# albcab/mfm

Measured on NVIDIA B200. Metric: chain-steps/sec (MALA+flow-MH+FM update), pines 40x40, higher is better.
Workload: dtype f32

## Files before the change

mfm_b200/csrc/flow.cu:

```cuda
#include "internal.h"
#include <limits.h>
#include <string.h>
#include <stdlib.h>
#include "gemm_tf32x3.cuh"
#include "ref_dist.cuh"

namespace mfm {

__constant__ float c_alpha[6] = {(float)(1.0 / 5), (float)(3.0 / 10), (float)(4.0 / 5), (float)(8.0 / 9), 1.0f, 1.0f};
__constant__ float c_beta[6][6] = {
    {(float)(1.0 / 5), 0, 0, 0, 0, 0},
    {(float)(3.0 / 40), (float)(9.0 / 40), 0, 0, 0, 0},
    {(float)(44.0 / 45), (float)(-56.0 / 15), (float)(32.0 / 9), 0, 0, 0},
    {(float)(19372.0 / 6561), (float)(-25360.0 / 2187), (float)(64448.0 / 6561), (float)(-212.0 / 729), 0, 0},
    {(float)(9017.0 / 3168), (float)(-355.0 / 33), (float)(46732.0 / 5247), (float)(49.0 / 176), (float)(-5103.0 / 18656), 0},
    {(float)(35.0 / 384), 0, (float)(500.0 / 1113), (float)(125.0 / 192), (float)(-2187.0 / 6784), (float)(11.0 / 84)}};
__constant__ float c_sol[7] = {(float)(35.0 / 384), 0, (float)(500.0 / 1113), (float)(125.0 / 192),
                               (float)(-2187.0 / 6784), (float)(11.0 / 84), 0};
__constant__ float c_err[7] = {(float)(35.0 / 384 - 1951.0 / 21600), 0, (float)(500.0 / 1113 - 22642.0 / 50085),
                               (float)(125.0 / 192 - 451.0 / 720), (float)(-2187.0 / 6784 - -12231.0 / 42400),
                               (float)(11.0 / 84 - 649.0 / 6300), (float)(-1.0 / 60.0)};
__constant__ float c_mid[7] = {(float)(6025192743.0 / 30085553152.0 / 2), 0, (float)(51252292925.0 / 65400821598.0 / 2),
                               (float)(-2691868925.0 / 45128329728.0 / 2), (float)(187940372067.0 / 1594534317056.0 / 2),
                               (float)(-1776094331.0 / 19743644256.0 / 2), (float)(11237099.0 / 235043384.0 / 2)};

struct EpiFieldV {
    static constexpr bool kRowSum = false;
    float* V; long long ldv; const float* bias; const float* gt; const float* gc; long long ld; float sgn;
    const int* row_map;
    float* amax_out = nullptr; mutable float vmax = 0.0f;
    struct Aux { float bias, gt, gc; int orow; };
    __device__ __forceinline__ Aux load(int row, int col) const {
        const long long o = (long long)row * ld + col;
        Aux a; a.bias = __ldg(bias + col); a.gt = __ldg(gt + o); a.gc = __ldg(gc + o);
        a.orow = row_map ? __ldg(row_map + row) : row;
        return a;
    }
    __device__ __forceinline__ float apply(int, int col, float acc, const Aux& a) const {
        const float v = sgn * (acc + a.bias + a.gt * a.gc);
        V[(long long)a.orow * ldv + col] = v; vmax = fmaxf(vmax, fabsf(v));
        return 0.0f;
    }
    __device__ __forceinline__ float operator()(int row, int col, float acc) const { return apply(row, col, acc, load(row, col)); }
    __device__ __forceinline__ void row_partial(int, int, float) const {}
    __device__ __forceinline__ void at_z(int) {}
    struct Col4 { float4 bias; };
    struct Row4 { float4 gt, gc; int orow; };
    bool vec_ok() const { return aligned16(V) && ldv % 4 == 0 && aligned16(bias) && aligned16(gt) && aligned16(gc) && ld % 4 == 0; }
    __device__ __forceinline__ Col4 load_col4(int col) const { Col4 c; c.bias = ldg4(bias + col); return c; }
    __device__ __forceinline__ Row4 load_row4(int row, int col) const {
        const long long o = (long long)row * ld + col;
        Row4 r; r.gt = ldg4(gt + o); r.gc = ldg4(gc + o); r.orow = row_map ? __ldg(row_map + row) : row;
        return r;
    }
    __device__ __forceinline__ float apply4(int, int col, const float4& acc, const Col4& c, const Row4& r) const {
        float4 v;
        v.x = sgn * (acc.x + c.bias.x + r.gt.x * r.gc.x); v.y = sgn * (acc.y + c.bias.y + r.gt.y * r.gc.y);
        v.z = sgn * (acc.z + c.bias.z + r.gt.z * r.gc.z); v.w = sgn * (acc.w + c.bias.w + r.gt.w * r.gc.w);
        st4(V + (long long)r.orow * ldv + col, v);
        vmax = amax4(vmax, v);
        return 0.0f;
    }
};
struct EpiFieldDiv {
    static constexpr bool kRowSum = true;
    const float* z; const float* gt; const float* hvc; long long ld; float* partial; int n_tiles;
    struct Aux { float z, gt, hvc; };
    __device__ __forceinline__ Aux load(int row, int col) const {
        const long long o = (long long)row * ld + col;
        Aux a; a.z = __ldg(z + o); a.gt = __ldg(gt + o); a.hvc = __ldg(hvc + o);
        return a;
    }
    __device__ __forceinline__ float apply(int, int, float acc, const Aux& a) const { return a.z * (acc + a.gt * a.hvc); }
    __device__ __forceinline__ float operator()(int row, int col, float acc) const { return apply(row, col, acc, load(row, col)); }
    struct Col4 {};
    struct Row4 { float4 z, gt, hvc; };
    bool vec_ok() const { return aligned16(z) && aligned16(gt) && aligned16(hvc) && ld % 4 == 0; }
    __device__ __forceinline__ Col4 load_col4(int) const { return Col4{}; }
    __device__ __forceinline__ Row4 load_row4(int row, int col) const {
        const long long o = (long long)row * ld + col;
        Row4 r; r.z = ldg4(z + o); r.gt = ldg4(gt + o); r.hvc = ldg4(hvc + o);
        return r;
    }
    __device__ __forceinline__ float apply4(int, int, const float4& acc, const Col4&, const Row4& r) const {
        return ((r.z.x * (acc.x + r.gt.x * r.hvc.x) + r.z.y * (acc.y + r.gt.y * r.hvc.y)) +
                (r.z.z * (acc.z + r.gt.z * r.hvc.z) + r.z.w * (acc.w + r.gt.w * r.hvc.w)));
    }
    __device__ __forceinline__ void row_partial(int row, int tile, float s) const { partial[(long long)row * n_tiles + tile] = s; }
    __device__ __forceinline__ void at_z(int) {}
};

int dense(int n, int in, int out, const float* A, long long lda, const float* WT, long long ldwt, const float* bias, int relu,
                 float* C, long long ldc, const float* mask, long long ldm, int mask_div, cudaStream_t st,
                 const int* n_rows_dev, DenseAmax am) {
    GemmShape p{n, out, in, A, lda, WT, ldwt, n_rows_dev};
    p.a_amax = am.a; p.a_amax2 = am.a2; p.a_bound = am.a_bound; p.a_split = am.a_split; p.a_scale_src = am.a_scale_src;
    const bool general = relu > ACT_RELU || am.dact != nullptr || am.mask_mul != 0;
    if (am.out_split && am.w_norm && (am.a || am.a_bound > 0.0f)) {
        auto run = [&](auto e) -> cudaError_t {
            e.alt_amax = am.alt_amax; e.alt_w_norm = am.alt_w_norm; e.alt_bias = am.alt_bias;
            e.amax_out = am.out; e.dact = am.dact; e.lddact = am.lddact; e.mask_mul = am.mask_mul;
            return launch_gemm<true, false>(p, e, st);
        };
        if (general) MFM_CUDA_CHECK(run(EpiStdSA{C, ldc, bias, mask, ldm, nullptr, 0, relu, mask_div, am.out_split, am.a, am.a2, am.a_bound, am.w_norm, am.bias_amax, am.add_bound, am.out_bound}));
        else MFM_CUDA_CHECK(run(EpiStdS{C, ldc, bias, mask, ldm, nullptr, 0, relu, mask_div, am.out_split, am.a, am.a2, am.a_bound, am.w_norm, am.bias_amax, am.add_bound, am.out_bound}));
        return MFM_OK;
// ... 582 lines not shown
                                                           int* __restrict__ n_active, long long* __restrict__ chain_evals) {
    __shared__ int wsum[32];
    __shared__ int total;
    const int per = (n + 1023) / 1024;
    const int b = threadIdx.x * per, e = min(n, b + per);
    int cnt = 0;
    for (int c = b; c < e; ++c) cnt += seg[c] < n_seg;
    const int lane = threadIdx.x & 31, w = threadIdx.x >> 5;
    int inc = cnt;
#pragma unroll
    for (int o = 1; o < 32; o <<= 1) { const int v = __shfl_up_sync(0xffffffffu, inc, o); if (lane >= o) inc += v; }
    if (lane == 31) wsum[w] = inc;
    __syncthreads();
    if (w == 0) {
        int v = wsum[lane], iv = v;
#pragma unroll
        for (int o = 1; o < 32; o <<= 1) { const int u = __shfl_up_sync(0xffffffffu, iv, o); if (lane >= o) iv += u; }
        wsum[lane] = iv - v;
        if (lane == 31) total = iv;
    }
    __syncthreads();
    int pos = wsum[w] + inc - cnt;
    for (int c = b; c < e; ++c) if (seg[c] < n_seg) idx[pos++] = c;
    if (threadIdx.x == 0) { *n_active = total; *chain_evals += 6ll * total; }
}

__global__ void ode_gather_probe_kernel(int n, int d, int H, const int* __restrict__ idx, const int* __restrict__ n_active,
                                        const float* __restrict__ z_full, const float* __restrict__ zw2_full,
                                        const float* __restrict__ zkinv_full, float* __restrict__ z, float* __restrict__ zw2,
                                        float* __restrict__ zkinv) {
    const int r = blockIdx.x;
    if (r >= min(n, *n_active)) return;
    const long long c = idx[r];
    for (int i = threadIdx.x; i < d; i += blockDim.x) {
        z[(long long)r * d + i] = z_full[c * d + i];
        if (zkinv_full) zkinv[(long long)r * d + i] = zkinv_full[c * d + i];
    }
    for (int i = threadIdx.x; i < H; i += blockDim.x) zw2[(long long)r * H + i] = zw2_full[c * H + i];
}

__device__ __forceinline__ float fit_eval(float y0, float y1, float ymid, float dy0, float dy1, float h, float rel) {
    const float a = -2.f * h * dy0 + 2.f * h * dy1 - 8.f * y0 - 8.f * y1 + 16.f * ymid;
    const float b = 5.f * h * dy0 - 3.f * h * dy1 + 18.f * y0 + 14.f * y1 - 32.f * ymid;
    const float c = -4.f * h * dy0 + h * dy1 - 11.f * y0 - 5.f * y1 + 16.f * ymid;
    const float dd = h * dy0;
    return (((a * rel + b) * rel + c) * rel + dd) * rel + y0;
}

}
#include "targets.cuh"
#include "ode_small.cuh"
namespace mfm {

__global__ void ode_finish_kernel(int n, int d, OdeState S, OdeTimes TS, float rtol, float atol, int mxstep) {
    const int lane = threadIdx.x & 31;
    const int c = blockIdx.x * (blockDim.x >> 5) + (threadIdx.x >> 5);
    if (c >= n) return;
    int seg = S.seg[c];
    if (seg >= TS.n_seg) return;
    const float tt = S.t[c], h = S.dt[c];
    const long long o = (long long)c * d;
    float sum = 0.0f;
    for (int i = lane; i < d; i += 32) {
        float ss = 0.0f, se = 0.0f;
#pragma unroll
        for (int j = 0; j < 7; ++j) { const float k = S.kx[j][o + i]; ss += c_sol[j] * k; se += c_err[j] * k; }
        const float y = S.yx[o + i];
        const float y1 = h * ss + y;
        const float r = (h * se) / (atol + rtol * fmaxf(fabsf(y), fabsf(y1)));
        sum += r * r;
    }
    float ssl = 0.0f, sel = 0.0f;
#pragma unroll
    for (int j = 0; j < 7; ++j) { const float k = S.kl[j][c]; ssl += c_sol[j] * k; sel += c_err[j] * k; }
    const float yl = S.yl[c];
    const float yl1 = h * ssl + yl;
    if (lane == 0) { const float r = (h * sel) / (atol + rtol * fmaxf(fabsf(yl), fabsf(yl1))); sum += r * r; }
    sum = warp_sum(sum);
    const float ratio = sqrtf(sum / (float)(d + 1));
    const bool accept = ratio <= 1.0f;
    float new_dt;
    if (isnan(ratio)) new_dt = NAN;
    else if (ratio == 0.0f) new_dt = h * 10.0f;
    else {
        const float dfac = ratio < 1.0f ? 1.0f : 0.2f;
        const float fac = fminf(10.0f, fmaxf(powf(ratio, -0.2f) * 0.9f, dfac));
        new_dt = h * fac;
    }
    if (new_dt < 0.0f) new_dt = 0.0f;
    float t_new = tt;
    if (accept) {
        t_new = tt + h;
        const float t_final = TS.target[TS.n_seg - 1];
        const float rel = (t_final - tt) / (t_new - tt);
        for (int i = lane; i < d; i += 32) {
            float ss = 0.0f, sm = 0.0f;
            float k0 = 0.f, k6 = 0.f;
#pragma unroll
            for (int j = 0; j < 7; ++j) {
                const float k = S.kx[j][o + i]; ss += c_sol[j] * k; sm += c_mid[j] * k;
                if (j == 0) k0 = k; if (j == 6) k6 = k;
            }
            const float y = S.yx[o + i];
            const float y1 = h * ss + y, ymid = y + h * sm;
            S.outx[o + i] = fit_eval(y, y1, ymid, k0, k6, h, rel);
            S.yx[o + i] = y1;
            S.kx[0][o + i] = k6;
        }
        if (lane == 0) {
            float sm = 0.0f;
#pragma unroll
            for (int j = 0; j < 7; ++j) sm += c_mid[j] * S.kl[j][c];
            S.outl[c] = fit_eval(yl, yl1, yl + h * sm, S.kl[0][c], S.kl[6][c], h, rel);
            S.yl[c] = yl1; S.kl[0][c] = S.kl[6][c]; S.t[c] = t_new;
        }
    }
    if (lane == 0) {
        int ic = S.icount[c] + 1;
        const int ntry = S.ntry[c] + 1;
        S.ntry[c] = ntry;
        S.dt[c] = new_dt;
        while (seg < TS.n_seg && !(t_new < TS.target[seg] && ic < mxstep && new_dt > 0.0f)) { ++seg; ic = 0; }
        S.seg[c] = seg; S.icount[c] = ic;
        if (seg < TS.n_seg) atomicAdd(&S.counters[0], 1);
        if (accept) atomicAdd(&S.counters[1], 1);
        atomicAdd(&S.counters[2], 1);
        atomicMax(&S.counters[3], ntry);
    }
}

__global__ void copy_out_kernel(int n, int d, const float* __restrict__ sx, const float* __restrict__ sl,
                                float* __restrict__ y1, float* __restrict__ ldj) {
    const long long i = blockIdx.x * (long long)blockDim.x + threadIdx.x;
    if (i < (long long)n * d) y1[i] = sx[i];
    if (i < n && ldj) ldj[i] = sl[i];
}

__global__ void write_stats_kernel(const int* __restrict__ counters, int n_eval, long long host_chain_evals, int* __restrict__ stats,
                                   int accumulate) {
    if (threadIdx.x == 0) {
        if (n_eval == INT_MIN) n_eval = 2 + 6 * counters[3];
        else if (n_eval < 0) n_eval = -n_eval + 6 * counters[12];
        if (host_chain_evals < 0) host_chain_evals = -host_chain_evals * n_eval;
        const long long ce = *reinterpret_cast<const long long*>(counters + 10) + host_chain_evals;
        long long* out_ce = reinterpret_cast<long long*>(stats + 4);
        if (accumulate) { stats[0] += counters[1]; stats[1] += counters[2]; stats[2] = max(stats[2], counters[3]); stats[3] += n_eval; *out_ce += ce; }
        else { stats[0] = counters[1]; stats[1] = counters[2]; stats[2] = counters[3]; stats[3] = n_eval; *out_ce = ce; stats[6] = 0; stats[7] = 0; }
    }
}

__global__ void ode_loop_cond_kernel(cudaGraphConditionalHandle handle, int* __restrict__ counters, long long max_iter) {
    if (threadIdx.x == 0) {
        const int it = ++counters[12];
        cudaGraphSetConditional(handle, (counters[0] > 0 && it < max_iter) ? 1u : 0u);
    }
}
struct OdeGraphKey {
    mfm_field_t F; mfm_target_t T; mfm_ode_opts_t O; int direction, n, flags; const void *z, *z_compact, *ws, *fb;
};
struct OdeGraphEntry { OdeGraphKey key; cudaGraph_t graph; cudaGraphExec_t exec; int dev; long long max_iter; unsigned long long stamp; bool used; };
static thread_local OdeGraphEntry g_ode_graphs[8];
static thread_local unsigned long long g_ode_graph_stamp = 0;
static int g_ode_small = -1;
static bool ode_small_enabled() {
    if (g_ode_small < 0) { const char* e = getenv("MFM_ODE_SMALL"); g_ode_small = (e && e[0] == '0') ? 0 : 1; }
    return g_ode_small != 0;
}
static int g_ode_graph_mode = -1;
static bool ode_use_graph(long long elements) {
    if (g_ode_graph_mode < 0) {
        const char* e = getenv("MFM_ODE_GRAPH");
        g_ode_graph_mode = (e && e[0] == '0') ? 0 : ((e && e[0] == '1') ? 1 : 2);
    }
    return g_ode_graph_mode == 1 || (g_ode_graph_mode == 2 && elements <= (4ll << 20));
}
// ... 84 lines not shown
    const int d = F.dim, H = F.hidden;
    const float sgn = direction >= 0 ? 1.0f : -1.0f;
    if (O.n_times < 2 || O.n_times > 17) { mfm_set_last_error_msg("n_times must be in [2,17]"); return MFM_ERR_ARG; }
    OdeTimes TS; TS.n_seg = O.n_times - 1;
    for (int k = 1; k < O.n_times; ++k) TS.target[k - 1] = (float)((double)k / (double)(O.n_times - 1));
    if (ode_small_enabled() && small::eligible(F, T, n)) {
        small::Args A;
        A.F = F; A.T = T; A.n = n; A.hutch = z != nullptr ? 1 : 0; A.n_seg = TS.n_seg;
        for (int k = 0; k < 16; ++k) A.target[k] = k < TS.n_seg ? TS.target[k] : 0.0f;
        A.rtol = O.rtol; A.atol = O.atol; A.mxstep = O.mxstep; A.sgn = sgn; A.y0 = y0; A.z = z; A.y1 = y1; A.ldj = ldj; A.counters = S.counters; A.wt = B.wt;
        static bool configured = false;
        if (!configured) {
            MFM_CUDA_CHECK(cudaFuncSetAttribute(small::ode_small_kernel, cudaFuncAttributeMaxDynamicSharedMemorySize, small::SMEM_BYTES));
            configured = true;
        }
        MFM_CUDA_CHECK(cudaMemsetAsync(S.counters, 0, 64 * sizeof(int), st));
        small::ode_small_kernel<<<ceil_div(n, small::CH), small::NTHR, small::SMEM_BYTES, st>>>(A);
        MFM_LAUNCH_CHECK();
        if (stats) { write_stats_kernel<<<1, 32, 0, st>>>(S.counters, INT_MIN, 0, stats, stats_accumulate); MFM_LAUNCH_CHECK(); }
        return MFM_OK;
    }
    int* hflag = host_flag();
    if (!hflag) { mfm_set_last_error_msg("cudaMallocHost failed"); return MFM_ERR_CUDA; }
    int rc;
    const int gE = ceil_div((long long)n * d, 256), gW = ceil_div(n, 8);
    const bool compact = z != nullptr;
    ode_init_kernel<<<max(gE, 1), 256, 0, st>>>(n, d, y0, S, 0.0f, sgn);
    MFM_LAUNCH_CHECK();
    if (z) {
        if ((rc = field_prepare_probe(F, T, n, z, B, st, z_bound))) return rc;
        if (compact) {
            MFM_CUDA_CHECK(cudaMemcpyAsync(S.zw2_full, B.zw2, (size_t)n * H * 4, cudaMemcpyDeviceToDevice, st));
            if (T.kind == MFM_TARGET_PINES)
                MFM_CUDA_CHECK(cudaMemcpyAsync(S.zkinv_full, B.zkinv, (size_t)n * d * 4, cudaMemcpyDeviceToDevice, st));
        }
    }
    int n_eval = 0;
    if ((rc = field_eval(F, T, n, S.xi, S.tf, z, sgn, S.kx[0], S.kl[0], B, st))) return rc; ++n_eval;
    ode_h0_kernel<<<gW, 256, 0, st>>>(n, d, S, O.rtol, O.atol, sgn);
    MFM_LAUNCH_CHECK();
    if ((rc = field_eval(F, T, n, S.xi, S.tf, z, sgn, S.kx[1], S.kl[1], B, st))) return rc; ++n_eval;
    ode_h1_kernel<<<gW, 256, 0, st>>>(n, d, S, O.rtol, O.atol);
    MFM_LAUNCH_CHECK();
    const int* idx = nullptr; const int* nact = nullptr; const float* zc = z;
    if (compact) {
        ode_compact_kernel<<<1, 1024, 0, st>>>(n, TS.n_seg, S.seg, S.idx, S.n_active, reinterpret_cast<long long*>(S.counters + 10));
        MFM_LAUNCH_CHECK();
        idx = S.idx; nact = S.n_active; zc = z_compact;
    }
    const long long max_iter = (long long)TS.n_seg * (long long)O.mxstep + 2;
    float* x_amax = (tc2h::gemm_h16() && B.amax && d % 16 == 0 && n >= 256) ? B.amax + AM_X : nullptr;
    bool stage_vec = d % 4 == 0 && ((reinterpret_cast<uintptr_t>(S.yx) | reinterpret_cast<uintptr_t>(S.xi)) & 15) == 0;
    for (int j = 0; j < 6; ++j) stage_vec = stage_vec && (reinterpret_cast<uintptr_t>(S.kx[j]) & 15) == 0;
    auto rk_iteration = [&](cudaStream_t s) -> int {
        int rc2;
        if (compact) {
            ode_gather_probe_kernel<<<n, 128, 0, s>>>(n, d, H, idx, nact, z, S.zw2_full,
                                                      T.kind == MFM_TARGET_PINES ? S.zkinv_full : nullptr, z_compact, B.zw2, B.zkinv);
            MFM_LAUNCH_CHECK();
        }
        for (int sg = 1; sg <= 6; ++sg) {
            if (stage_vec) ode_stage4_kernel<<<ceil_div((long long)n * (d / 4), 256), 256, 0, s>>>(n, d / 4, sg, S, TS.n_seg, sgn, idx, nact, x_amax);
            else ode_stage_kernel<<<gE, 256, 0, s>>>(n, d, sg, S, TS.n_seg, sgn, idx, nact, x_amax);
            MFM_LAUNCH_CHECK();
            if ((rc2 = field_eval(F, T, n, S.xi, S.tf, zc, sgn, S.kx[sg], S.kl[sg], B, s, nact, idx, x_amax))) return rc2;
        }
        MFM_CUDA_CHECK(cudaMemsetAsync(S.counters, 0, sizeof(int), s));
        ode_finish_kernel<<<gW, 256, 0, s>>>(n, d, S, TS, O.rtol, O.atol, O.mxstep);
        MFM_LAUNCH_CHECK();
        if (compact) {
            ode_compact_kernel<<<1, 1024, 0, s>>>(n, TS.n_seg, S.seg, S.idx, S.n_active, reinterpret_cast<long long*>(S.counters + 10));
            MFM_LAUNCH_CHECK();
        }
        return MFM_OK;
    };
    bool looped_on_device = false;
    if (ode_use_graph((long long)n * d)) {
        OdeGraphKey key;
        memset(&key, 0, sizeof(key));
        key.F = F; key.T = T; key.T.beta = 0.0f; key.O = O; key.direction = direction; key.n = n; key.z = z; key.z_compact = z_compact;
        key.ws = S.z_full; key.fb = B.ff; key.flags = tc2h::gemm_h16() * 16 + tc2h::split_groups() + 64 * gemm_backend();
        rc = ode_graph_launch(key, st, S.counters, max_iter, rk_iteration);
        if (rc == MFM_OK) looped_on_device = true;
        else if (rc != MFM_ERR_UNSUPPORTED) return rc;
    }
    if (!looped_on_device)
    for (long long it = 0; it < max_iter; ++it) {
        if ((rc = rk_iteration(st))) return rc;
        n_eval += 6;
        MFM_CUDA_CHECK(cudaMemcpyAsync(hflag, S.counters, sizeof(int), cudaMemcpyDeviceToHost, st));
        MFM_CUDA_CHECK(cudaStreamSynchronize(st));
        if (*hflag == 0) break;
    }
    copy_out_kernel<<<max(gE, 1), 256, 0, st>>>(n, d, S.outx, S.outl, y1, ldj);
    MFM_LAUNCH_CHECK();
    if (stats) {
        const long long host_ce = compact ? 2ll * n : (looped_on_device ? -(long long)n : (long long)n * n_eval);
        write_stats_kernel<<<1, 32, 0, st>>>(S.counters, looped_on_device ? -n_eval : n_eval, host_ce, stats, stats_accumulate); MFM_LAUNCH_CHECK();
    }
    return MFM_OK;
}

__global__ void flow_keys_kernel(const uint32_t* __restrict__ rng_key, int n, int chain_offset, int n_total,
                                 uint32_t* __restrict__ kgen, uint32_t* __restrict__ kacc, uint32_t* __restrict__ kh1,
                                 uint32_t* __restrict__ kh2) {
    const int c = blockIdx.x * blockDim.x + threadIdx.x;
    if (c >= n) return;
    u32x2 kc;
    if (n_total > 0) kc = threefry_split_key(rng_key[0], rng_key[1], (uint32_t)(chain_offset + c), (uint32_t)n_total);
    else { kc.a = rng_key[2 * c]; kc.b = rng_key[2 * c + 1]; }
    uint32_t* outs[4] = {kgen, kacc, kh1, kh2};
#pragma unroll
    for (int j = 0; j < 4; ++j) {
        const u32x2 k = threefry_split_key(kc.a, kc.b, (uint32_t)j, 4u);
        outs[j][2 * c] = k.a; outs[j][2 * c + 1] = k.b;
    }
}

__global__ void axpy_kernel(long long total, const float* __restrict__ a, float scale, const float* __restrict__ eps,
                            float* __restrict__ out) {
    const long long i = blockIdx.x * (long long)blockDim.x + threadIdx.x;
// ... 377 lines not shown
```

mfm_b200/csrc/gemm_tcgen05_h16.cuh:

```cuda
#pragma once
#include <cuda_fp16.h>
#include "gemm_tcgen05_persist.cuh"

namespace mfm {
namespace tc2h {

using namespace tc2p;
__device__ __forceinline__ void mma_f16_ss_2sm(uint32_t d, uint64_t a, uint64_t b, uint32_t idesc, uint32_t acc) { mma_bf16_ss_2sm(d, a, b, idesc, acc); }

constexpr int S_STAGES = 6, S_STAGE_BYTES = HI_BYTES;
constexpr int S_NBARS = 3 * S_STAGES + 4;
constexpr int S_SMEM_BYTES = S_STAGES * S_STAGE_BYTES + EPI_STG_BYTES + 1024  + 256 ;
static_assert(S_NBARS * 8 + 8 + 64 <= 256, "barrier area: barriers, TMEM slot, PairWork");
static_assert(S_STAGE_BYTES == EPI_WARPS * 4096, "the helpers' staging is exactly ring stage 0");

__host__ __device__ __forceinline__ uint32_t h16_scale_exp(float amax) {
#ifdef __CUDA_ARCH__
    const uint32_t b = __float_as_uint(amax) & 0x7FFFFFFFu;
#else
    union { float f; uint32_t u; } c; c.f = amax; const uint32_t b = c.u & 0x7FFFFFFFu;
#endif
    int e = (int)(b >> 23);
    if (b == 0u || e == 255) return 127u;
    if (e == 0) e = 1;
// ... 185 lines not shown
        }
    } else if (warp >= SPLIT_WARP0 && warp < EPI_WARP0) {
        const int G = (APRE && BPRE) ? 1 : sc.split_groups, per_group = SPLIT_WARPS * 32 / G;
        const int tix = threadIdx.x - SPLIT_WARP0 * 32;
        const int grp = tix / per_group, tg = tix - grp * per_group;
        const float s_a = APRE ? 1.0f : h16_scale(h16_a_amax(sc)), s_b = BPRE ? 1.0f : h16_scale(*sc.b_amax);
        uint32_t g = 0;
        for (int idx = 0; idx < work->n_items; ++idx) {
            int tile, kb0, kb1;
            item_at(idx, tile, kb0, kb1);
            int n_kb = kb1 - kb0;
            if (p.k_split > 0) { int m0p, n0, kz0, KT, neff, z; tile_origin(tile, m0p, n0, kz0, KT, neff, z); n_kb = KT; }
            for (int kt = 0; kt < n_kb; ++kt, ++g) {
                if ((int)(g % (uint32_t)G) != grp) continue;
                const uint32_t s = g % S_STAGES, ph = (g / S_STAGES) & 1;
                mbar_wait(&full[s], ph);
                if (APRE && BPRE) {
                    if (warp == SPLIT_WARP0 && lane == 0) mbar_arrive_remote(&split[s], 0);
                    continue;
                }
#pragma unroll 1
                for (int un = (APRE ? 256 : 0) + tg; un < (BPRE ? 256 : 512) && !(APRE && BPRE); un += per_group) {
                    const int op = un >> 8;
                    const uint32_t r = ((uint32_t)un & 255u) >> 1, hq = (uint32_t)un & 1u;
                    const uint32_t rowa = smem_u32(smem + s * S_STAGE_BYTES) + (op ? A_BYTES : 0) + r * 128u;
                    float4 v[4];
#pragma unroll
                    for (int j = 0; j < 4; ++j)
                        asm volatile("ld.shared.v4.f32 {%0, %1, %2, %3}, [%4];" : "=f"(v[j].x), "=f"(v[j].y), "=f"(v[j].z), "=f"(v[j].w)
                                     : "r"(rowa + (((4u * hq + (uint32_t)j) ^ (r & 7u)) << 4)));
                    uint32_t hp[8], lp[8];
                    if (sc.cvt_unpack) split16<true>(v, op ? s_b : s_a, hp, lp); else split16<false>(v, op ? s_b : s_a, hp, lp);
#pragma unroll
                    for (int j = 0; j < 2; ++j) {
                        asm volatile("st.shared.v4.b32 [%0], {%1, %2, %3, %4};" ::"r"(rowa + (((4u * hq + (uint32_t)j) ^ (r & 7u)) << 4)),
                                     "r"(hp[4 * j]), "r"(hp[4 * j + 1]), "r"(hp[4 * j + 2]), "r"(hp[4 * j + 3]) : "memory");
                        asm volatile("st.shared.v4.b32 [%0], {%1, %2, %3, %4};" ::"r"(rowa + (((4u * hq + 2u + (uint32_t)j) ^ (r & 7u)) << 4)),
                                     "r"(lp[4 * j]), "r"(lp[4 * j + 1]), "r"(lp[4 * j + 2]), "r"(lp[4 * j + 3]) : "memory");
                    }
                }
                asm volatile("fence.proxy.async.shared::cta;" ::: "memory");
                __syncwarp();
                if (lane == 0) mbar_arrive_remote(&split[s], 0);
            }
        }
    }
    if (warp >= SPLIT_WARP0) {
        const bool helper = warp < EPI_WARP0;
        const int ew = helper ? warp - SPLIT_WARP0 : warp - EPI_WARP0;
        const int quad = ew & 3;
        const int chalf = ew >> 2;
        const uint32_t stg = helper ? smem_u32(smem) + (uint32_t)ew * 4096u : smem_u32(stg_base) + (uint32_t)ew * 4096u;
        const int rsub = lane >> 3, cpiece = (lane & 7) * 4;
        constexpr int RB = sizeof(typename Epi::Row4) > 36 ? 2 : 4;
        const float inv_s = h16_inv_scale(APRE ? *sc.a_scale_src : h16_a_amax(sc)) * h16_inv_scale(*sc.b_amax);
        float vmax = 0.0f;
        if (work->n_head != 0 && (!helper || work->n_items == 1)) {
            int tile, kb0_, kb1_, m0p, n0, kz0, KT, neff, z;
            item_at(0, tile, kb0_, kb1_);
            tile_origin(tile, m0p, n0, kz0, KT, neff, z);
            const int n_chunks = min(BN / 32, (p.N - n0 + 31) / 32);
            int cc_begin = chalf * 4, cc_end = min(n_chunks, chalf * 4 + 4);
            if (work->n_items == 1) { if (helper) cc_begin = min(cc_begin + 2, cc_end); else cc_end = min(cc_end, cc_begin + 2); }
            mbar_wait(&acc_full[0], 0);
            asm volatile("tcgen05.fence::after_thread_sync;" ::: "memory");
            if (ew == 0 && !helper) TC2P_MARKX(48);
            if (cc_begin >= cc_end && !helper) {
                asm volatile("tcgen05.fence::before_thread_sync;" ::: "memory");
                __syncwarp();
                if (lane == 0) mbar_arrive_remote(&acc_empty[0], 0);
            }
#pragma unroll 1
            for (int cc = cc_begin; cc < cc_end; ++cc) {
                uint32_t r[32];
                tmem_ld32_nowait(tmem_base + ((uint32_t)(quad * 32) << 16) + (uint32_t)(cc * 32), r);
                asm volatile("tcgen05.wait::ld.sync.aligned;" ::: "memory");
                if (cc == cc_end - 1 && !helper) {
                    asm volatile("tcgen05.fence::before_thread_sync;" ::: "memory");
                    __syncwarp();
                    if (lane == 0) mbar_arrive_remote(&acc_empty[0], 0);
                }
                const uint32_t dst = stg + (uint32_t)lane * 128u;
#pragma unroll
                for (int j = 0; j < 8; ++j)
                    asm volatile("st.shared.v4.f32 [%0], {%1, %2, %3, %4};" ::"r"(dst + (uint32_t)((j ^ (lane & 7)) << 4)), "f"(__uint_as_float(r[4 * j])),
                                 "f"(__uint_as_float(r[4 * j + 1])), "f"(__uint_as_float(r[4 * j + 2])), "f"(__uint_as_float(r[4 * j + 3])) : "memory");
                __syncwarp();
                float* dstp = sk_ws + (size_t)pair * SK_SLOT_FLOATS + (size_t)((int)rank * BM + quad * 32 + rsub) * BN + cc * 32 + cpiece;
                const uint32_t sa = stg + (uint32_t)rsub * 128u;
#pragma unroll
                for (int k = 0; k < 8; ++k) {
                    float4 v;
                    asm volatile("ld.shared.v4.f32 {%0, %1, %2, %3}, [%4];" : "=f"(v.x), "=f"(v.y), "=f"(v.z), "=f"(v.w)
                                 : "r"(sa + (uint32_t)k * 512u + (uint32_t)(((lane & 7) ^ ((k * 4 + rsub) & 7)) << 4)));
                    __stcg(reinterpret_cast<float4*>(dstp + (size_t)k * 4 * BN), v);
                }
            }
            __syncwarp();
            if (lane == 0) {
                __threadfence();
                for (int cc = cc_begin; cc < cc_end; ++cc)
                    asm volatile("st.relaxed.gpu.global.u32 [%0], %1;" ::"l"(sk_flags + (size_t)pair * SK_SLOT_FLAGS + rank * 32u + (uint32_t)quad * 8u + (uint32_t)cc),
                                 "r"(sk_epoch) : "memory");
            }
        }
        if (ew == 0 && !helper) TC2P_MARKX(49);
        uint32_t i = (uint32_t)(helper ? max(work->n_items - 1, work->n_head) : work->n_head);
        for (; (int)i < work->n_items; ++i) {
            int tile, kb0_, kb1_, m0p, n0, kz0, KT, neff, z;
            item_at((int)i, tile, kb0_, kb1_);
            tile_origin(tile, m0p, n0, kz0, KT, neff, z);
            const uint32_t b = i & 1, u = i >> 1;
            const bool last = (int)i == work->n_items - 1;
            const bool fix = work->fix != 0 && (int)i == work->n_head;
            Epi e = epi;
            if (p.k_split > 0) e.at_z(z);
            const int row_base = m0p + (int)rank * BM + quad * 32;
            const int n_chunks = min(BN / 32, (p.N - n0 + 31) / 32);
            int cc_begin = chalf * 4, cc_end = min(n_chunks, chalf * 4 + 4);
            if (last) { if (helper) cc_begin = min(cc_begin + 2, cc_end); else cc_end = min(cc_end, cc_begin + 2); }
            mbar_wait(&acc_full[b], u & 1);
            asm volatile("tcgen05.fence::after_thread_sync;" ::: "memory");
            if (ew == 0 && !helper) TC2P_MARK(i, 2);
            float rs[8];
#pragma unroll
            for (int k = 0; k < 8; ++k) rs[k] = 0.0f;
            if (cc_begin >= cc_end && !helper) {
                asm volatile("tcgen05.fence::before_thread_sync;" ::: "memory");
                __syncwarp();
                if (lane == 0) mbar_arrive_remote(&acc_empty[b], 0);
            }
#pragma unroll 1
            for (int cc = cc_begin; cc < cc_end; ++cc) {
                const int col0 = cc * 32;
                uint32_t r[32];
                tmem_ld32_nowait(tmem_base + ((uint32_t)(quad * 32) << 16) + b * BN + (uint32_t)col0, r);
                asm volatile("tcgen05.wait::ld.sync.aligned;" ::: "memory");
                if (cc == cc_end - 1 && !helper) {
                    asm volatile("tcgen05.fence::before_thread_sync;" ::: "memory");
                    __syncwarp();
                    if (lane == 0) mbar_arrive_remote(&acc_empty[b], 0);
                }
                const uint32_t dst = stg + (uint32_t)lane * 128u;
#pragma unroll
                for (int j = 0; j < 8; ++j)
                    asm volatile("st.shared.v4.f32 [%0], {%1, %2, %3, %4};" ::"r"(dst + (uint32_t)((j ^ (lane & 7)) << 4)), "f"(__uint_as_float(r[4 * j])),
                                 "f"(__uint_as_float(r[4 * j + 1])), "f"(__uint_as_float(r[4 * j + 2])), "f"(__uint_as_float(r[4 * j + 3])) : "memory");
                __syncwarp();
                if (fix) {
                    const int c_first = work->last.c_first, c_count = work->last.c_count;
                    const uint32_t fidx = rank * 32u + (uint32_t)quad * 8u + (uint32_t)cc;
                    if (lane < c_count) {
                        const unsigned* fl = sk_flags + (size_t)(c_first + lane) * SK_SLOT_FLAGS + fidx;
                        unsigned seen;
                        do {
                            asm volatile("ld.acquire.gpu.global.u32 %0, [%1];" : "=r"(seen) : "l"(fl) : "memory");
                        } while (seen != sk_epoch);
                    }
                    __syncwarp();
                    const size_t toff = (size_t)((int)rank * BM + quad * 32 + rsub) * BN + col0 + cpiece;
                    const uint32_t sa = stg + (uint32_t)rsub * 128u;
#pragma unroll 1
                    for (int c = 0; c < c_count; ++c) {
                        const float* srcp = sk_ws + (size_t)(c_first + c) * SK_SLOT_FLOATS + toff;
                        float4 v[8];
#pragma unroll
                        for (int k = 0; k < 8; ++k) v[k] = __ldcg(reinterpret_cast<const float4*>(srcp + (size_t)k * 4 * BN));
#pragma unroll
                        for (int k = 0; k < 8; ++k) {
                            const uint32_t ad = sa + (uint32_t)k * 512u + (uint32_t)(((lane & 7) ^ ((k * 4 + rsub) & 7)) << 4);
                            float4 w;
                            asm volatile("ld.shared.v4.f32 {%0, %1, %2, %3}, [%4];" : "=f"(w.x), "=f"(w.y), "=f"(w.z), "=f"(w.w) : "r"(ad));
                            asm volatile("st.shared.v4.f32 [%0], {%1, %2, %3, %4};" ::"r"(ad), "f"(w.x + v[k].x), "f"(w.y + v[k].y), "f"(w.z + v[k].z), "f"(w.w + v[k].w) : "memory");
// ... 134 lines not shown
```

mfm_b200/csrc/gemm_tf32x3.cuh:

```cuda
#pragma once
#include "common.cuh"
#include <cuda_fp16.h>

namespace mfm {

constexpr int GBM = 128, GBN = 64, GBK = 16, GSTAGES = 3, GTHREADS = 256;
constexpr int G_MI = 2, G_NJ = 4;
constexpr int G_FLUSH = 2;
constexpr int LDS_K = GBK + 4;
constexpr int LDS_AM = GBM + 8;
constexpr int LDS_BN = GBN + 8;
constexpr int A_STAGE = (GBM * LDS_K > GBK * LDS_AM) ? GBM * LDS_K : GBK * LDS_AM;
constexpr int B_STAGE = (GBN * LDS_K > GBK * LDS_BN) ? GBN * LDS_K : GBK * LDS_BN;
constexpr int GEMM_SMEM_BYTES = GSTAGES * (A_STAGE + B_STAGE) * 4 + GBM * 2 * 4;

struct GemmShape {
    int M, N, K;
    const float* A; long long lda;
    const float* B; long long ldb;
    const int* n_rows_dev;
    int k_split = 0;
    const float* a_amax = nullptr;
    const float* a_amax2 = nullptr;
    float a_bound = 0.0f;
    const float* b_amax = nullptr;
    const float* b_mirror = nullptr;
    const float* a_split = nullptr;
    const float* a_scale_src = nullptr;
};

template <class E> __device__ __forceinline__ auto epi_stored_max(const E& e, int) -> decltype(e.vmax) { return e.vmax; }
template <class E> __device__ __forceinline__ float epi_stored_max(const E&, long) { return 0.0f; }
template <class E> __device__ __forceinline__ auto epi_amax_slot(const E& e, int) -> decltype(e.amax_out) { return e.amax_out; }
template <class E> __device__ __forceinline__ float* epi_amax_slot(const E&, long) { return nullptr; }
template <class E> __device__ __forceinline__ auto epi_publish_bound(const E& e, int) -> decltype((void)e.bound_out) {
    if (blockIdx.x == 0 && blockIdx.y == 0 && blockIdx.z == 0 && (threadIdx.x & 31) == 0 && e.bound_out) *e.bound_out = e.out_bound();
}
template <class E> __device__ __forceinline__ void epi_publish_bound(const E&, long) {}
template <class E, class = void> struct epi_has_colsum { static constexpr bool value = false; };
template <class E> struct epi_has_colsum<E, decltype((void)E::kColSum)> { static constexpr bool value = E::kColSum; };
template <class E> __device__ __forceinline__ void epi_publish_amax(const E& e, float vmax) {
    float* slot = epi_amax_slot(e, 0);
    if (slot != nullptr) amax_publish_warp(slot, vmax);
    epi_publish_bound(e, 0);
}

__device__ __forceinline__ void cp_async16(void* smem, const void* gmem, bool pred) {
    const uint32_t s = (uint32_t)__cvta_generic_to_shared(smem);
    const int sz = pred ? 16 : 0;
    asm volatile("cp.async.cg.shared.global [%0], [%1], 16, %2;\n" ::"r"(s), "l"(gmem), "r"(sz));
}
__device__ __forceinline__ void cp_async_commit() { asm volatile("cp.async.commit_group;\n" ::); }
template <int N> __device__ __forceinline__ void cp_async_wait() { asm volatile("cp.async.wait_group %0;\n" ::"n"(N)); }

__device__ __forceinline__ uint32_t f2tf32(float x) {
    uint32_t r; asm("cvt.rna.tf32.f32 %0, %1;\n" : "=r"(r) : "f"(x)); return r;
}
__device__ __forceinline__ void split_tf32(float x, uint32_t& hi, uint32_t& lo) {
    hi = f2tf32(x);
    lo = f2tf32(x - __uint_as_float(hi));
}
__device__ __forceinline__ void mma_tf32(float (&c)[4], const uint32_t (&a)[4], const uint32_t (&b)[2]) {
    asm volatile("mma.sync.aligned.m16n8k8.row.col.f32.tf32.tf32.f32 {%0,%1,%2,%3}, {%4,%5,%6,%7}, {%8,%9}, {%0,%1,%2,%3};\n"
                 : "+f"(c[0]), "+f"(c[1]), "+f"(c[2]), "+f"(c[3])
                 : "r"(a[0]), "r"(a[1]), "r"(a[2]), "r"(a[3]), "r"(b[0]), "r"(b[1]));
}

template <bool KMAJ, int ROWS, int LDS_R>
__device__ __forceinline__ void load_tile(float* s, const float* __restrict__ g, long long ld, int row0, int k0,
                                          int rows, int K, bool vec_ok) {
    const int tid = threadIdx.x;
    constexpr int CHUNKS = ROWS * GBK / 4;
#pragma unroll
    for (int it = 0; it < (CHUNKS + GTHREADS - 1) / GTHREADS; ++it) {
        const int c = tid + it * GTHREADS;
        if (CHUNKS % GTHREADS != 0 && c >= CHUNKS) break;
        int r, kk, nr, nk;
        float* dst;
        if (KMAJ) { r = c >> 2; kk = (c & 3) * 4; nr = 1; nk = 4; dst = s + r * LDS_K + kk; }
        else      { kk = c / (ROWS / 4); r = (c % (ROWS / 4)) * 4; nr = 4; nk = 1; dst = s + kk * LDS_R + r; }
        const int gr = row0 + r, gk = k0 + kk;
        const bool full = (gr + nr <= rows) && (gk + nk <= K);
        const bool none = (gr >= rows) || (gk >= K);
        if (vec_ok && (full || none)) {
            const float* src = full ? (KMAJ ? g + (long long)gr * ld + gk : g + (long long)gk * ld + gr) : g;
            cp_async16(dst, src, full);
            continue;
        }
#pragma unroll
        for (int e = 0; e < 4; ++e) {
            const int er = KMAJ ? gr : gr + e, ek = KMAJ ? gk + e : gk;
            dst[e] = (er < rows && ek < K) ? (KMAJ ? g[(long long)er * ld + ek] : g[(long long)ek * ld + er]) : 0.0f;
        }
// ... 408 lines not shown
```

Measured before the change: 2.305 million.

## Restructure ODE step-finish into block-per-chain kernel with smem stash and L2 prefetch

The ODE finish kernel changes from one warp per chain to one block per chain. It uses float4 loads, computes the mid-point interpolant in the same first pass, and stashes results in shared memory so the accept pass does not re-read the seven stage buffers. It also launches only the active compacted chains through the index list. Separately, the field-V GEMM epilogue gets a fixed row batch of 4 and issues bulk L2 prefetches of its gt/gc operands before waiting on the accumulator. The trade-off is more shared memory, small blocks when d is small (d=1600 here), and a stash path that depends on alignment.

```diff
diff --git a/mfm_b200/csrc/flow.cu b/mfm_b200/csrc/flow.cu
--- a/mfm_b200/csrc/flow.cu
+++ b/mfm_b200/csrc/flow.cu
@@ -26,6 +26,8 @@
 
 struct EpiFieldV {
     static constexpr bool kRowSum = false;
+    static constexpr bool kPrefetch = true;
+    static constexpr int kRowBatch = 4;
     float* V; long long ldv; const float* bias; const float* gt; const float* gc; long long ld; float sgn;
     const int* row_map;
     float* amax_out = nullptr; mutable float vmax = 0.0f;
@@ -52,6 +54,10 @@
         const long long o = (long long)row * ld + col;
         Row4 r; r.gt = ldg4(gt + o); r.gc = ldg4(gc + o); r.orow = row_map ? __ldg(row_map + row) : row;
         return r;
+    }
+    __device__ __forceinline__ void prefetch_l2(int row, int col, int bytes) const {
+        const long long o = (long long)row * ld + col;
+        mfm::prefetch_l2(gt + o, bytes); mfm::prefetch_l2(gc + o, bytes);
     }
     __device__ __forceinline__ float apply4(int, int col, const float4& acc, const Col4& c, const Row4& r) const {
         float4 v;
@@ -740,32 +746,70 @@
 #include "ode_small.cuh"
 namespace mfm {
 
-__global__ void ode_finish_kernel(int n, int d, OdeState S, OdeTimes TS, float rtol, float atol, int mxstep) {
-    const int lane = threadIdx.x & 31;
-    const int c = blockIdx.x * (blockDim.x >> 5) + (threadIdx.x >> 5);
-    if (c >= n) return;
+static constexpr long long FINISH_SMEM_MAX = 200 * 1024;
+template <int V>
+__global__ void __launch_bounds__(256) ode_finish_kernel(int n, int d, OdeState S, OdeTimes TS, float rtol, float atol, int mxstep,
+                                                         const int* __restrict__ idx, const int* __restrict__ n_active, int stash) {
+    extern __shared__ float fsm[];
+    float* s_r = fsm; float* s_out = fsm + d; float* s_y1 = s_out + d; float* s_k6 = s_y1 + d;
+    __shared__ float s_sum;
+    if (idx && (int)blockIdx.x >= min(n, *n_active)) return;
+    const int c = idx ? idx[blockIdx.x] : (int)blockIdx.x;
     int seg = S.seg[c];
     if (seg >= TS.n_seg) return;
     const float tt = S.t[c], h = S.dt[c];
+    const float t_new = tt + h;
+    const float rel = (TS.target[TS.n_seg - 1] - tt) / (t_new - tt);
     const long long o = (long long)c * d;
-    float sum = 0.0f;
-    for (int i = lane; i < d; i += 32) {
-        float ss = 0.0f, se = 0.0f;
+    auto load = [&](const float* p, int i, float* v) {
+        if constexpr (V == 4) { const float4 q = __ldg(reinterpret_cast<const float4*>(p + o + i)); v[0] = q.x; v[1] = q.y; v[2] = q.z; v[3] = q.w; }
+        else v[0] = p[o + i];
+    };
+    auto store = [&](float* p, int i, const float* v) {
+        if constexpr (V == 4) *reinterpret_cast<float4*>(p + o + i) = make_float4(v[0], v[1], v[2], v[3]);
+        else p[o + i] = v[0];
+    };
+    auto step = [&](int i, float* r, float* y1, float* out, float* k6) {
+        float k[7][V], y[V];
 #pragma unroll
-        for (int j = 0; j < 7; ++j) { const float k = S.kx[j][o + i]; ss += c_sol[j] * k; se += c_err[j] * k; }
-        const float y = S.yx[o + i];
-        const float y1 = h * ss + y;
-        const float r = (h * se) / (atol + rtol * fmaxf(fabsf(y), fabsf(y1)));
-        sum += r * r;
-    }
-    float ssl = 0.0f, sel = 0.0f;
+        for (int j = 0; j < 7; ++j) load(S.kx[j], i, k[j]);
+        load(S.yx, i, y);
 #pragma unroll
-    for (int j = 0; j < 7; ++j) { const float k = S.kl[j][c]; ssl += c_sol[j] * k; sel += c_err[j] * k; }
+        for (int e = 0; e < V; ++e) {
+            float ss = 0.0f, se = 0.0f, sm = 0.0f;
+#pragma unroll
+            for (int j = 0; j < 7; ++j) { ss += c_sol[j] * k[j][e]; se += c_err[j] * k[j][e]; sm += c_mid[j] * k[j][e]; }
+            y1[e] = h * ss + y[e];
+            r[e] = (h * se) / (atol + rtol * fmaxf(fabsf(y[e]), fabsf(y1[e])));
+            out[e] = fit_eval(y[e], y1[e], y[e] + h * sm, k[0][e], k[6][e], h, rel);
+            k6[e] = k[6][e];
+        }
+    };
+    for (int i = threadIdx.x * V; i < d; i += blockDim.x * V) {
+        float r[V], y1[V], out[V], k6[V];
+        step(i, r, y1, out, k6);
+#pragma unroll
+        for (int e = 0; e < V; ++e) {
+            s_r[i + e] = r[e];
+            if (stash) { s_out[i + e] = out[e]; s_y1[i + e] = y1[e]; s_k6[i + e] = k6[e]; }
+        }
+    }
+    float ssl = 0.0f, sel = 0.0f, sml = 0.0f;
+#pragma unroll
+    for (int j = 0; j < 7; ++j) { const float k = S.kl[j][c]; ssl += c_sol[j] * k; sel += c_err[j] * k; sml += c_mid[j] * k; }
     const float yl = S.yl[c];
     const float yl1 = h * ssl + yl;
-    if (lane == 0) { const float r = (h * sel) / (atol + rtol * fmaxf(fabsf(yl), fabsf(yl1))); sum += r * r; }
-    sum = warp_sum(sum);
-    const float ratio = sqrtf(sum / (float)(d + 1));
+    __syncthreads();
+    if (threadIdx.x < 32) {
+        const int lane = threadIdx.x;
+        float sum = 0.0f;
+        for (int i = lane; i < d; i += 32) { const float r = s_r[i]; sum += r * r; }
+        if (lane == 0) { const float r = (h * sel) / (atol + rtol * fmaxf(fabsf(yl), fabsf(yl1))); sum += r * r; }
+        sum = warp_sum(sum);
+        if (lane == 0) s_sum = sum;
+    }
+    __syncthreads();
+    const float ratio = sqrtf(s_sum / (float)(d + 1));
     const bool accept = ratio <= 1.0f;
     float new_dt;
     if (isnan(ratio)) new_dt = NAN;
@@ -776,39 +820,31 @@
         new_dt = h * fac;
     }
     if (new_dt < 0.0f) new_dt = 0.0f;
-    float t_new = tt;
     if (accept) {
-        t_new = tt + h;
-        const float t_final = TS.target[TS.n_seg - 1];
-        const float rel = (t_final - tt) / (t_new - tt);
-        for (int i = lane; i < d; i += 32) {
-            float ss = 0.0f, sm = 0.0f;
-            float k0 = 0.f, k6 = 0.f;
+        for (int i = threadIdx.x * V; i < d; i += blockDim.x * V) {
+            float r[V], y1[V], out[V], k6[V];
+            if (stash) {
 #pragma unroll
-            for (int j = 0; j < 7; ++j) {
-                const float k = S.kx[j][o + i]; ss += c_sol[j] * k; sm += c_mid[j] * k;
-                if (j == 0) k0 = k; if (j == 6) k6 = k;
+                for (int e = 0; e < V; ++e) { out[e] = s_out[i + e]; y1[e] = s_y1[i + e]; k6[e] = s_k6[i + e]; }
+            } else {
+                step(i, r, y1, out, k6);
             }
-            const float y = S.yx[o + i];
-            const float y1 = h * ss + y, ymid = y + h * sm;
-            S.outx[o + i] = fit_eval(y, y1, ymid, k0, k6, h, rel);
-            S.yx[o + i] = y1;
-            S.kx[0][o + i] = k6;
-        }
-        if (lane == 0) {
-            float sm = 0.0f;
-#pragma unroll
-            for (int j = 0; j < 7; ++j) sm += c_mid[j] * S.kl[j][c];
-            S.outl[c] = fit_eval(yl, yl1, yl + h * sm, S.kl[0][c], S.kl[6][c], h, rel);
+            store(S.outx, i, out);
+            store(S.yx, i, y1);
+            store(S.kx[0], i, k6);
+        }
+    }
+    if (threadIdx.x == 0) {
+        const float t_out = accept ? t_new : tt;
+        if (accept) {
+            S.outl[c] = fit_eval(yl, yl1, yl + h * sml, S.kl[0][c], S.kl[6][c], h, rel);
             S.yl[c] = yl1; S.kl[0][c] = S.kl[6][c]; S.t[c] = t_new;
         }
-    }
-    if (lane == 0) {
         int ic = S.icount[c] + 1;
         const int ntry = S.ntry[c] + 1;
         S.ntry[c] = ntry;
         S.dt[c] = new_dt;
-        while (seg < TS.n_seg && !(t_new < TS.target[seg] && ic < mxstep && new_dt > 0.0f)) { ++seg; ic = 0; }
+        while (seg < TS.n_seg && !(t_out < TS.target[seg] && ic < mxstep && new_dt > 0.0f)) { ++seg; ic = 0; }
         S.seg[c] = seg; S.icount[c] = ic;
         if (seg < TS.n_seg) atomicAdd(&S.counters[0], 1);
         if (accept) atomicAdd(&S.counters[1], 1);
@@ -999,6 +1035,15 @@
     float* x_amax = (tc2h::gemm_h16() && B.amax && d % 16 == 0 && n >= 256) ? B.amax + AM_X : nullptr;
     bool stage_vec = d % 4 == 0 && ((reinterpret_cast<uintptr_t>(S.yx) | reinterpret_cast<uintptr_t>(S.xi)) & 15) == 0;
     for (int j = 0; j < 6; ++j) stage_vec = stage_vec && (reinterpret_cast<uintptr_t>(S.kx[j]) & 15) == 0;
+    const bool fin_vec = stage_vec && ((reinterpret_cast<uintptr_t>(S.kx[6]) | reinterpret_cast<uintptr_t>(S.outx)) & 15) == 0;
+    const int fin_thr = (int)min(256ll, max(32ll, ceil_div(ceil_div((long long)d, fin_vec ? 4 : 1), 32) * 32ll));
+    const int fin_stash = 16ll * d <= FINISH_SMEM_MAX ? 1 : 0;
+    const size_t fin_smem = (size_t)d * sizeof(float) * (fin_stash ? 4 : 1);
+    if (fin_smem > FINISH_SMEM_MAX) { mfm_set_last_error_msg("ODE: dim too large for the step-finish kernel"); return MFM_ERR_UNSUPPORTED; }
+    if (fin_smem > 48 * 1024) {
+        MFM_CUDA_CHECK(cudaFuncSetAttribute(ode_finish_kernel<4>, cudaFuncAttributeMaxDynamicSharedMemorySize, (int)fin_smem));
+        MFM_CUDA_CHECK(cudaFuncSetAttribute(ode_finish_kernel<1>, cudaFuncAttributeMaxDynamicSharedMemorySize, (int)fin_smem));
+    }
     auto rk_iteration = [&](cudaStream_t s) -> int {
         int rc2;
         if (compact) {
@@ -1013,7 +1058,8 @@
             if ((rc2 = field_eval(F, T, n, S.xi, S.tf, zc, sgn, S.kx[sg], S.kl[sg], B, s, nact, idx, x_amax))) return rc2;
         }
         MFM_CUDA_CHECK(cudaMemsetAsync(S.counters, 0, sizeof(int), s));
-        ode_finish_kernel<<<gW, 256, 0, s>>>(n, d, S, TS, O.rtol, O.atol, O.mxstep);
+        if (fin_vec) ode_finish_kernel<4><<<n, fin_thr, fin_smem, s>>>(n, d, S, TS, O.rtol, O.atol, O.mxstep, idx, nact, fin_stash);
+        else ode_finish_kernel<1><<<n, fin_thr, fin_smem, s>>>(n, d, S, TS, O.rtol, O.atol, O.mxstep, idx, nact, fin_stash);
         MFM_LAUNCH_CHECK();
         if (compact) {
             ode_compact_kernel<<<1, 1024, 0, s>>>(n, TS.n_seg, S.seg, S.idx, S.n_active, reinterpret_cast<long long*>(S.counters + 10));
diff --git a/mfm_b200/csrc/gemm_tcgen05_h16.cuh b/mfm_b200/csrc/gemm_tcgen05_h16.cuh
--- a/mfm_b200/csrc/gemm_tcgen05_h16.cuh
+++ b/mfm_b200/csrc/gemm_tcgen05_h16.cuh
@@ -261,7 +261,7 @@
         const int chalf = ew >> 2;
         const uint32_t stg = helper ? smem_u32(smem) + (uint32_t)ew * 4096u : smem_u32(stg_base) + (uint32_t)ew * 4096u;
         const int rsub = lane >> 3, cpiece = (lane & 7) * 4;
-        constexpr int RB = sizeof(typename Epi::Row4) > 36 ? 2 : 4;
+        constexpr int RB = epi_row_batch<Epi>::value;
         const float inv_s = h16_inv_scale(APRE ? *sc.a_scale_src : h16_a_amax(sc)) * h16_inv_scale(*sc.b_amax);
         float vmax = 0.0f;
         if (work->n_head != 0 && (!helper || work->n_items == 1)) {
@@ -328,6 +328,10 @@
             const int n_chunks = min(BN / 32, (p.N - n0 + 31) / 32);
             int cc_begin = chalf * 4, cc_end = min(n_chunks, chalf * 4 + 4);
             if (last) { if (helper) cc_begin = min(cc_begin + 2, cc_end); else cc_end = min(cc_end, cc_begin + 2); }
+            if constexpr (epi_has_prefetch<Epi>::value) {
+                const int prow = row_base + lane, pcol = n0 + cc_begin * 32;
+                if (prow < M && cc_begin < cc_end && pcol < p.N) e.prefetch_l2(prow, pcol, 4 * (min(n0 + cc_end * 32, p.N) - pcol));
+            }
             mbar_wait(&acc_full[b], u & 1);
             asm volatile("tcgen05.fence::after_thread_sync;" ::: "memory");
             if (ew == 0 && !helper) TC2P_MARK(i, 2);
diff --git a/mfm_b200/csrc/gemm_tf32x3.cuh b/mfm_b200/csrc/gemm_tf32x3.cuh
--- a/mfm_b200/csrc/gemm_tf32x3.cuh
+++ b/mfm_b200/csrc/gemm_tf32x3.cuh
@@ -39,6 +39,13 @@
 template <class E> __device__ __forceinline__ void epi_publish_bound(const E&, long) {}
 template <class E, class = void> struct epi_has_colsum { static constexpr bool value = false; };
 template <class E> struct epi_has_colsum<E, decltype((void)E::kColSum)> { static constexpr bool value = E::kColSum; };
+template <class E, class = void> struct epi_row_batch { static constexpr int value = sizeof(typename E::Row4) > 36 ? 2 : 4; };
+template <class E> struct epi_row_batch<E, decltype((void)E::kRowBatch)> { static constexpr int value = E::kRowBatch; };
+template <class E, class = void> struct epi_has_prefetch { static constexpr bool value = false; };
+template <class E> struct epi_has_prefetch<E, decltype((void)E::kPrefetch)> { static constexpr bool value = E::kPrefetch; };
+__device__ __forceinline__ void prefetch_l2(const void* p, int bytes) {
+    asm volatile("cp.async.bulk.prefetch.L2.global [%0], %1;" ::"l"(p), "r"(bytes) : "memory");
+}
 template <class E> __device__ __forceinline__ void epi_publish_amax(const E& e, float vmax) {
     float* slot = epi_amax_slot(e, 0);
     if (slot != nullptr) amax_publish_warp(slot, vmax);
```

After: 2.328 million, median of 6. Within noise of the previous version (+1.0%).
